# jgsimard/big-dreamer

Hardware: AMD Instinct MI355X
Metric: latent transitions/sec (RSSM + imagination) at batch=50 chunk=50 H=15 (higher is better)
Workload: dtype f32

## Files before the change

### big_dreamer_amd/_cabi.py

```python
from __future__ import annotations

import ctypes as C
import os

import torch

_HERE = os.path.dirname(os.path.abspath(__file__))
LIB_PATH = os.environ.get("BD_LIB") or os.path.join(_HERE, "libbigdreamer_hip.so")

if not os.path.exists(LIB_PATH):
    raise ImportError(
        f"{LIB_PATH} is missing: the MI355X HIP extension has not been built "
        "(run `python -c 'import __graft_entry__ as g; g.build()'`). There is no CPU fallback.")

lib = C.CDLL(LIB_PATH)

BD_MAX_LAYERS = 6
ACT_NONE, ACT_ELU, ACT_ELU_GRAD = 0, 1, 2
ACT_RELU, ACT_RELU_GRAD, ACT_TANH, ACT_TANH_GRAD = 3, 4, 5, 6
CNN_ACTS = {"ELU": (ACT_ELU, ACT_ELU_GRAD), "ReLU": (ACT_RELU, ACT_RELU_GRAD), "Tanh": (ACT_TANH, ACT_TANH_GRAD)}
GRAD_ACTS = (ACT_ELU_GRAD, ACT_RELU_GRAD, ACT_TANH_GRAD)
P = C.c_void_p
F32 = C.c_float
I32 = C.c_int
# ... 197 lines not shown
    "bd_rng_fill": (I32, [C.POINTER(RngFillArgs), P]),
    "bd_philox4x32_10": (I32, [C.POINTER(C.c_uint), C.POINTER(C.c_uint), C.POINTER(C.c_uint)]),
    "bd_actor_entropy_rng": (I32, [C.c_ulonglong, C.c_ulonglong, C.c_uint, P, P, I32, I32, I32, I32, P]),
    "bd_gemm_nt": (I32, [P, I32, P, I32, P, I32, I32, I32, I32, I32, P]),
    "bd_categorical_head_forward": (I32, [P, P, I32, I32, I32, P, P, P]),
    "bd_categorical_head_backward": (I32, [P, P, I32, I32, I32, P, P]),
    "bd_kl_categorical_forward": (I32, [P, P, I32, I32, I32, F32, I32, P, I32, P, P]),
    "bd_kl_categorical_backward": (I32, [P, P, I32, I32, I32, F32, F32, F32, F32, P, I32, P, P, P]),
    "bd_plan_rollout": (I32, [C.POINTER(PlanArgs), P]),
    "bd_cem_refit": (I32, [P, I32, P, I32, I32, I32, I32, I32, P, P, P]),
    "bd_plan_rollout_cat": (I32, [C.POINTER(PlanCatArgs), P]),
    "bd_lambda_return_backward": (I32, [P, F32, I32, I32, F32, F32, P, P, P]),
    "bd_img_heads_supported": (I32, [I32, I32]),
    "bd_img_heads_fwd_bwd": (I32, [C.POINTER(ImgHeadsArgs), P]),
    "bd_actor_reinforce": (I32, [P, P, P, P, P, P, P, I32, I32, I32, F32, F32, F32, I32, P, P, I32, P, P]),
    "bd_actor_reinforce_cat": (I32, [P, P, P, P, P, P, I32, I32, I32, F32, F32, F32, I32, P, P, I32, P, P]),
    "bd_normal_nll": (I32, [P, I32, P, I32, I32, I32, F32, P, I32, P, I32, P, P]),
    "bd_bernoulli_nll": (I32, [P, P, C.c_size_t, F32, P, P, I32, P, P]),
    "bd_kl_forward": (I32, [P, P, P, P, I32, I32, F32, I32, P, I32, P, P]),
    "bd_kl_backward": (I32, [P, P, P, P, I32, I32, F32, F32, F32, F32, P, I32, P, P, P, P, P]),
    "bd_sum": (I32, [P, C.c_size_t, P, I32, P, P]),
    "bd_sumsq": (I32, [P, C.c_size_t, P, I32, P, P]),
    "bd_adam_step": (I32, [P, P, P, P, C.c_size_t, F32, F32, F32, F32, F32, I32, F32, P, I32, P]),
    "bd_polyak": (I32, [P, P, C.c_size_t, F32, P]),
    "bd_replay_gather": (I32, [P, P, I32, I32, P, P]),
    "bd_replay_gather_pixels": (I32, [P, P, I32, I32, I32, P, P, P]),
    "bd_replay_gather_pixels_rng": (I32, [P, P, I32, I32, I32, C.c_ulonglong, C.c_ulonglong, P, P]),
    "bd_reduce_ws_floats": (C.c_size_t, []),
    "bd_conv_gemm": (I32, [C.POINTER(ConvArgs), P]),
    "bd_conv_thin_forward": (I32, [P, I32, I32, I32, I32, I32, P, I32, P, I32, P, P, P]),
    "bd_conv_pack_class": (I32, [P, P, I32, I32, I32, I32, I32, I32, I32, P]),
    "bd_conv_pack_fused": (I32, [P, P, I32, I32, I32, P]),
    "bd_act_backward": (I32, [P, P, C.c_size_t, I32, P]),
    "bd_elu_backward": (I32, [P, P, C.c_size_t, P]),
    "bd_image_layout": (I32, [P, P, I32, I32, I32, I32, P]),
    "bd_colsum_ws_floats": (C.c_size_t, [I32]),
    "bd_colsum": (I32, [P, C.c_size_t, I32, P, P, P]),
}

for _name, (_res, _args) in _SIGS.items():
    _fn = getattr(lib, _name)
    _fn.restype = _res
    _fn.argtypes = _args

EXPORTED = tuple(_SIGS)

# ... 24 lines not shown
```

### big_dreamer_amd/csrc/cabi.hip

```cpp
#include "bd_device.h"
#include "bd_host.h"
#include "bd_rng.h"

namespace bd {
char* err_buf() {
    static thread_local char buf[512] = "";
    return buf;
}

__global__ __launch_bounds__(256) void pack_kernel(const bd_pack_desc* __restrict__ descs) {
    const bd_pack_desc d = descs[blockIdx.y];
    const int No = d.transpose ? d.K : d.N;
    const int Ki = d.transpose ? d.N : d.K;
    const int Nb = (No + 15) >> 4, Kb = (Ki + 15) >> 4;
    const int total = Nb * Kb * 64;
    floatx4* __restrict__ dst = reinterpret_cast<floatx4*>(d.dst);
    for (int e = blockIdx.x * blockDim.x + threadIdx.x; e < total; e += gridDim.x * blockDim.x) {
        const int lane = e & 63, blk = e >> 6;
        const int nb = blk / Kb, kb = blk - nb * Kb;
        const int n = nb * 16 + (lane & 15);
        const int k0 = kb * 16 + 4 * (lane >> 4);
        floatx4 v;
#pragma unroll
        for (int i = 0; i < 4; ++i) {
            const int k = k0 + i;
            float x = 0.f;
            if (n < No && k < Ki) x = d.transpose ? d.src[(size_t)k * d.ld + n] : d.src[(size_t)n * d.ld + k];
            v[i] = x;
        }
        dst[e] = v;
    }
}

__global__ __launch_bounds__(256) void gather_rows_kernel(const float* __restrict__ src, const int64_t* __restrict__ idx,
                                                          int n_idx, int width, float* __restrict__ dst) {
    const size_t total = (size_t)n_idx * width;
    for (size_t e = (size_t)blockIdx.x * blockDim.x + threadIdx.x; e < total; e += (size_t)gridDim.x * blockDim.x) {
        const size_t r = e / width, c = e - r * width;
        dst[e] = src[(size_t)idx[r] * width + c];
    }
}
template <bool RNG>
__global__ __launch_bounds__(256) void gather_pixels_kernel(const unsigned char* __restrict__ src,
                                                            const int64_t* __restrict__ idx, int n_idx, int pixels,
                                                            float inv_q, float inv_b, const float* __restrict__ noise,
                                                            float* __restrict__ dst, Rng rng) {
    const int quads = pixels >> 2;
    const size_t total = (size_t)n_idx * quads;
    for (size_t e = (size_t)blockIdx.x * blockDim.x + threadIdx.x; e < total; e += (size_t)gridDim.x * blockDim.x) {
        const size_t r = e / quads, q = e - r * quads;
        const uchar4 u = reinterpret_cast<const uchar4*>(src + (size_t)idx[r] * pixels)[q];
        floatx4 nz;
        if constexpr (RNG) {
            const Philox4 p = philox4x32_10((uint32_t)e, (uint32_t)(e >> 32), rng.stream, rng.step, rng.k0, rng.k1);
// ... 65 lines not shown
```

### big_dreamer_amd/csrc/reduce.hip

```cpp
#include "bd_device.h"
#include "bd_host.h"
#include "bd_discrete.h"

namespace bd {

constexpr int kRedBlocks = 1024;
constexpr float kHalfLog2Pi = 0.91893853320467274178f;

static inline int red_blocks(size_t n) {
    size_t b = (n + 255) / 256;
    return (int)(b < 1 ? 1 : (b > kRedBlocks ? kRedBlocks : b));
}

__global__ __launch_bounds__(256) void final_sum_kernel(const double* __restrict__ partials, int n,
                                                        float* __restrict__ scalars, int slot) {
    __shared__ double red[kWaves];
    double s = 0.0;
    for (int i = threadIdx.x; i < n; i += blockDim.x) s += partials[i];
    s = block_sum_d(s, red);
    if (threadIdx.x == 0) scalars[slot] = (float)s;
}

template <int MODE>
__global__ __launch_bounds__(256) void sum_kernel(const float* __restrict__ x, size_t n, double* __restrict__ partials) {
    __shared__ double red[kWaves];
// ... 131 lines not shown
    const size_t n = (size_t)M * S;
    for (size_t i = (size_t)blockIdx.x * blockDim.x + threadIdx.x; i < n; i += (size_t)gridDim.x * blockDim.x) {
        const size_t r = i / S, c = i - r * S;
        const float ds = dstate ? dstate[i] : 0.f;
        const float gm = ds + (dmean ? dmean[i] : 0.f);
        const float gs = (dstate ? ds * eps[i] : 0.f) + (dstd ? dstd[i] : 0.f);
        dout[r * 2 * S + c] = gm;
        dout[r * 2 * S + S + c] = gs * sigmoidf(out[r * 2 * S + S + c]);
    }
}

__global__ __launch_bounds__(256) void lambda_fwd_kernel(const float* __restrict__ reward, const float* __restrict__ value,
                                                         int Hm, int N, float disc, float lam, float* __restrict__ ret) {
    const float one_minus = 1.f - lam, dl = disc * lam;
    for (int n = blockIdx.x * blockDim.x + threadIdx.x; n < N; n += gridDim.x * blockDim.x) {
        const float boot = value[(size_t)(Hm - 1) * N + n];
        float last = boot;
        for (int t = Hm - 1; t >= 0; --t) {
            const float next = (t == Hm - 1) ? boot : value[(size_t)(t + 1) * N + n];
            const float inp = reward[(size_t)t * N + n] + disc * next * one_minus;
            last = inp + dl * last;
            ret[(size_t)t * N + n] = last;
        }
    }
}

__global__ __launch_bounds__(256) void lambda_bwd_kernel(const float* __restrict__ dret, float dconst, int Hm, int N,
                                                         float disc, float lam, float* __restrict__ dreward,
                                                         float* __restrict__ dvalue) {
    const float c = disc * lam, w = disc * (1.f - lam);
    for (int n = blockIdx.x * blockDim.x + threadIdx.x; n < N; n += gridDim.x * blockDim.x) {
        float G = 0.f;
        for (int t = 0; t < Hm; ++t) {
            G = (dret ? dret[(size_t)t * N + n] : dconst) + c * G;
            dreward[(size_t)t * N + n] = G;
            if (t == 0 && Hm > 1) dvalue[n] = 0.f;
            if (t < Hm - 1) {
                dvalue[(size_t)(t + 1) * N + n] = G * w;
            } else {
                const float prev = (Hm > 1) ? dvalue[(size_t)t * N + n] : 0.f;
                dvalue[(size_t)t * N + n] = prev + G * w + c * G;
            }
        }
    }
}

// ... 53 lines not shown
        const float w = weight ? weight[i] : 1.f;
        const float adv = ret[i] - (i < N ? base0[i] : value[i - N]);
        const float c = scale * w * adv;
        const size_t j = (size_t)i * A + lane;
        const float norm = valid ? stats[j] : -INFINITY;
        const unsigned long long hot = __ballot(valid && action[j] > 0.5f);
        const int k = hot ? __builtin_ctzll(hot) : 0;
        const float p = disc_probs(norm, valid);
        const float l = __shfl(norm, k, 64);
        float g = c * ((lane == k ? 1.f : 0.f) - p);
        if (write) {
            const float H = disc_entropy(norm, p, valid);
            g += (dentropy * w) * (-p * (norm + H));
        } else if (valid) {
            g += dout[j];
        }
        if (valid) dout[j] = g;
        if (lane == 0) s += (double)(w * l * adv);
    }
    s = block_sum_d(s, red);
    if (threadIdx.x == 0) partials[blockIdx.x] = s;
}

__global__ __launch_bounds__(256) void adam_kernel(float* __restrict__ p, float* __restrict__ g, float* __restrict__ m,
                                                   float* __restrict__ v, size_t n, float beta1, float beta2, float eps,
                                                   float wd, float step_size, float inv_sqrt_bc2, float max_norm,
                                                   const float* __restrict__ scalars, int sqnorm_slot) {
    const float total_norm = sqrtf(scalars[sqnorm_slot]);
    const float q = max_norm / (total_norm + 1e-6f);
    const float coef = q > 1.f ? 1.f : q;
    for (size_t i = (size_t)blockIdx.x * blockDim.x + threadIdx.x; i < n; i += (size_t)gridDim.x * blockDim.x) {
        const float gc = g[i] * coef;
        g[i] = gc;
        const float pi = p[i];
        const float gw = gc + wd * pi;
        const float mi = m[i] + (1.f - beta1) * (gw - m[i]);
        const float vi = v[i] * beta2 + (1.f - beta2) * gw * gw;
        m[i] = mi;
        v[i] = vi;
        const float denom = sqrtf(vi) * inv_sqrt_bc2 + eps;
        p[i] = pi - step_size * (mi / denom);
    }
}

__global__ __launch_bounds__(256) void polyak_kernel(float* __restrict__ t, const float* __restrict__ s, size_t n, float w) {
    for (size_t i = (size_t)blockIdx.x * blockDim.x + threadIdx.x; i < n; i += (size_t)gridDim.x * blockDim.x)
        t[i] = s[i] * w + t[i] * (1.f - w);
}

constexpr int kCatPer = 4;

__device__ __forceinline__ float half_max(float v) {
#pragma unroll
    for (int o = 16; o > 0; o >>= 1) v = fmaxf(v, __shfl_xor(v, o, 64));
    return v;
}
__device__ __forceinline__ float half_sum(float v) {
#pragma unroll
    for (int o = 16; o > 0; o >>= 1) v += __shfl_xor(v, o, 64);
    return v;
}

__device__ __forceinline__ void group_log_softmax(const float* __restrict__ x, int C, int l, float (&lp)[kCatPer]) {
    float m = -INFINITY;
// ... 296 lines not shown
    BD_CHECK_LAUNCH("bd_lambda_return_forward");
    return 0;
}

int bd_lambda_return_backward(const float* dreturns, float dret_const, int Hm, int N, float discount, float lambda_,
                              float* dreward, float* dvalue, void* stream) {
    BD_REQUIRE(dreward && dvalue && Hm > 0 && N > 0, "bd_lambda_return_backward: bad arguments");
    hipLaunchKernelGGL(lambda_bwd_kernel, dim3(red_blocks(N)), dim3(256), 0, (hipStream_t)stream, dreturns, dret_const, Hm,
                       N, discount, lambda_, dreward, dvalue);
    BD_CHECK_LAUNCH("bd_lambda_return_backward");
    return 0;
}

int bd_adam_step(float* p, float* g, float* m, float* v, size_t n, float lr, float beta1, float beta2, float eps,
                 float weight_decay, int step, float max_norm, const float* scalars, int sqnorm_slot, void* stream) {
    BD_REQUIRE(p && g && m && v && scalars && n > 0 && step >= 1, "bd_adam_step: bad arguments");
    const double bc1 = 1.0 - pow((double)beta1, step), bc2 = 1.0 - pow((double)beta2, step);
    hipLaunchKernelGGL(adam_kernel, dim3(red_blocks(n)), dim3(256), 0, (hipStream_t)stream, p, g, m, v, n, beta1, beta2,
                       eps, weight_decay, (float)(lr / bc1), (float)(1.0 / sqrt(bc2)), max_norm, scalars, sqnorm_slot);
    BD_CHECK_LAUNCH("bd_adam_step");
    return 0;
}

int bd_polyak(float* target, const float* src, size_t n, float weight, void* stream) {
    BD_REQUIRE(target && src && n > 0, "bd_polyak: bad arguments");
    hipLaunchKernelGGL(polyak_kernel, dim3(red_blocks(n)), dim3(256), 0, (hipStream_t)stream, target, src, n, weight);
    BD_CHECK_LAUNCH("bd_polyak");
    return 0;
}

static inline int cat_blocks(size_t units) {
    size_t b = (units + 7) / 8;
    return (int)(b < 1 ? 1 : (b > (size_t)kRedBlocks ? (size_t)kRedBlocks : b));
}

int bd_categorical_head_forward(const float* logits, const float* q_noise, int rows, int D, int C, float* state,
                                float* probs, void* stream) {
    BD_REQUIRE(logits && q_noise && state && probs && rows > 0 && D > 0, "bd_categorical_head_forward: bad arguments");
    BD_REQUIRE(C > 0 && C <= 32 * kCatPer, "bd_categorical_head_forward: %d classes (max %d)", C, 32 * kCatPer);
    const size_t groups = (size_t)rows * D;
    hipLaunchKernelGGL(cat_head_fwd_kernel, dim3(cat_blocks(groups)), dim3(256), 0, (hipStream_t)stream, logits, q_noise,
                       groups, C, state, probs);
    BD_CHECK_LAUNCH("bd_categorical_head_forward");
    return 0;
}

// ... 38 lines not shown
```

### big_dreamer_amd/engine.py

```python
from __future__ import annotations

import collections.abc
import ctypes as C
import math
import os
import weakref
from typing import Dict, List, Optional, Tuple

import numpy as np
import torch

from . import _cabi as cabi
from .parallel import DataParallel
from .params import ParamGroup, _adam_state_dict, _load_adam_state_dict
from .synth import CNN_ACTIVATIONS, DENSE_LAYERS, MODEL_MODULES, Dims, model_modules, param_shapes

lib = cabi.lib
ptr = cabi.ptr

DEFAULT_HP = dict(
    kl_balance=0.8, kl_loss_weight=0.1, free_nats=3.0, grad_clip_norm=100.0, discount=0.995, disclam=0.95,
    model_learning_rate=2e-4, actor_learning_rate=4e-5, value_learning_rate=1e-4, adam_epsilon=1e-5,
    weight_decay=1e-6, entropy_weight=1e-5, polyak_avg=1.0, min_std_dev=0.1, discount_weight=5.0,
    gradient_mixing=-1,
)

ACT_RAW_INIT_STD = float(torch.log(torch.exp(torch.tensor(5.0)) - 1))
ACT_MIN_STD = 1e-4
ACT_MEAN_SCALE = 5.0

SLOT_OBS, SLOT_REW, SLOT_KL, SLOT_RET, SLOT_ENT, SLOT_VAL, SLOT_GN_MODEL, SLOT_GN_ACTOR, SLOT_GN_CRITIC = range(9)
SLOT_DISC, SLOT_WOBJ = 9, 10
SLOT_RF = 11
N_SLOTS = 16


def check_gradient_mixing(value) -> float:
    try:
        rho = float(value)
    except (TypeError, ValueError):
        raise ValueError(f"gradient_mixing must be -1 or a number in [0, 1], got {value!r}") from None
    if not (rho == -1 or 0.0 <= rho <= 1.0):
        raise ValueError(f"gradient_mixing must be -1 or a number in [0, 1], got {value!r}")
    return rho


def check_cnn_activation(value) -> str:
    if value not in CNN_ACTIVATIONS:
        raise ValueError(f"cnn_activation_function must be one of {CNN_ACTIVATIONS}, got {value!r}")
    return value


def check_dense_activation(value) -> str:
    if value != "ELU":
        raise NotImplementedError("the HIP path implements the reference default activation (ELU)")
    return value
# ... 135 lines not shown
            tiny = torch.zeros(4, dtype=torch.float32, device=self.dev)
            for g in (None, "model", "actor", "critic"):
                self.dp.allreduce_sum_(tiny, g)
            torch.cuda.synchronize(self.dev)
        d = dims
        shapes = param_shapes(d)
        self.groups = {
            "model": ParamGroup([(m, n, s) for m in model_modules(d) for n, s in shapes[m]], self.dev,
                                conv_storage=self.pixel),
            "actor": ParamGroup([("actor", n, s) for n, s in shapes["actor"]], self.dev),
            "critic": ParamGroup([("critic", n, s) for n, s in shapes["critic"]], self.dev),
            "critic_target": ParamGroup([("critic_target", n, s) for n, s in shapes["critic"]], self.dev, False),
        }
        self._mod_group = {m: "model" for m in model_modules(d)}
        self._mod_group.update(actor="actor", critic="critic", critic_target="critic_target")
        if params is not None:
            self.load_params(params)
        self.scalars = torch.zeros(N_SLOTS, dtype=torch.float32, device=self.dev)
        self.red_ws = torch.zeros(int(lib.bd_reduce_ws_floats()), dtype=torch.float32, device=self.dev)
        self._wgrad_ws = torch.zeros(1, dtype=torch.float32, device=self.dev)
        self._wgrad_ws_side = torch.zeros(1, dtype=torch.float32, device=self.dev)
        self._wgrad_ws_early = torch.zeros(1, dtype=torch.float32, device=self.dev)
        self.red_ws_side = torch.zeros(int(lib.bd_reduce_ws_floats()), dtype=torch.float32, device=self.dev)
        self._wbatch = {"model": WgradBatch(self, "model"), "model_early": WgradBatch(self, "model_early", "_wgrad_ws_early"),
                        "actor": WgradBatch(self, "actor", "_wgrad_ws_bh"),
                        "critic": WgradBatch(self, "critic", "_wgrad_ws_side")}
        self._side = _engine_stream(self.dev, "side", int(os.environ.get("BD_SIDE_PRIO", "0")))
        self.heads_fused = (os.environ.get("BD_HEADS_FUSED", "1") != "0" and not self.d.categorical
                            and bool(lib.bd_img_heads_supported(self.d.Be + self.d.S, self.d.Hd)))
        self._s_early = _engine_stream(self.dev, "early", int(os.environ.get("BD_EARLY_PRIO", "0")))
        self.pipeline = os.environ.get("BD_PIPELINE", "1") != "0"
        self._s_wm = _engine_stream(self.dev, "wm", int(os.environ.get("BD_WM_PRIO", "-1")))
        bh_prio = int(os.environ.get("BD_BH_PRIO", "0" if self.pixel else "-1"))
        self._s_bh = _engine_stream(self.dev, "bh", bh_prio)
        self._ev_bh_wm_free: Optional[torch.cuda.Event] = None
        self._ev_bh_done: List[Optional[torch.cuda.Event]] = [None, None]
        self._ev_cr_done: List[Optional[torch.cuda.Event]] = [None, None]
        shared_comm = not all(g in self.dp.groups for g in ("model", "actor", "critic"))
        self.defer_opt = (world_size > 1 and shared_comm) or os.environ.get("BD_DEFER_OPT", "0") == "1"
        if os.environ.get("BD_FORCE_DP", "0") == "1" and torch.distributed.is_initialized():
            self.dp.force = True
            self.defer_opt = shared_comm or os.environ.get("BD_DEFER_OPT", "0") == "1"
        if (world_size > 1 or self.dp.force) and torch.cuda.current_stream(self.dev) == torch.cuda.default_stream(self.dev):
            self._main_stream = _engine_stream(self.dev, "main", 0)
            torch.cuda.set_stream(self._main_stream)
        self._pending_opt: List[tuple] = []
# ... 168 lines not shown
        if d.discrete_actions:
            add("actor", "a4", Wa4, tr=True)
        else:
            add("actor", "a4m", Wa4[:A], tr=True)
            add("actor", "a4s", Wa4[A:], tr=True)
            add("actor", "a4", Wa4, fwd=False, tr=True)

        self.pk: Dict[str, torch.Tensor] = {}
        self._pack_tables = {}
        for group, lst in ent.items():
            total = sum(cabi.packed_floats(*(v.shape if not tr else v.shape[::-1])) for _, v, tr in lst)
            store = torch.zeros(total, dtype=torch.float32, device=self.dev)
            descs = (cabi.PackDesc * len(lst))()
            off = 0
            for i, (key, v, tr) in enumerate(lst):
                N, K = v.shape
                n = cabi.packed_floats(N, K)
                self.pk[key] = store[off:off + n]
                descs[i] = cabi.PackDesc(v.data_ptr(), self.pk[key].data_ptr(), v.stride(0), N, K, int(tr))
                off += n
            raw = torch.frombuffer(bytearray(bytes(descs)), dtype=torch.uint8).to(self.dev)
            self._pack_tables[group] = (raw, len(lst), store)

    def pack(self, group: str) -> None:
        raw, n, _ = self._pack_tables[group]
        cabi.check(lib.bd_pack_weights(raw.data_ptr(), n, cabi.stream()))
        for dst, src, grp in self._plain.values():
            if grp == group:
                dst.copy_(src.t())
        if group == "model" and self.conv is not None:
            self.conv.pack()

    def _dense_spec(self, mod: str, prefix: str, in_width: int, out_width: int):
        sizes = [in_width] + [self.d.Hd] * DENSE_LAYERS + [out_width]
        return [(f"{prefix}{l}", self.W(mod, f"model.{2 * l}.bias"), sizes[l + 1], sizes[l],
                 cabi.ACT_ELU if l < DENSE_LAYERS else cabi.ACT_NONE) for l in range(DENSE_LAYERS + 1)]

    def mlp_forward(self, M, in0, ld0, w0, layers, saves, out, ldo, in1=None, ld1=0, w1=0, raw_packs=False,
                    gather=None) -> None:
        a = cabi.MlpFwdArgs()
        a.M, a.in0, a.ld0, a.w0 = M, ptr(in0), ld0, w0
        a.in1, a.ld1, a.w1 = ptr(in1), ld1, w1
        if gather is not None:
            a.gidx, a.gWT, a.gD, a.gC = ptr(gather[0]), ptr(gather[1]), gather[2], gather[3]
        a.n_layers = len(layers)
        for i, (key, bias, N, K, act) in enumerate(layers):
            a.layer[i] = cabi.Layer(ptr(key if raw_packs else self.pk[key]), ptr(bias), N, K, act,
                                    ptr(saves[i]) if saves else None)
        a.out, a.ldo = ptr(out), ldo
# ... 21 lines not shown
        cabi.check(lib.bd_wgrad(ptr(dpre), ldp, ptr(act), lda, M, N, K, ptr(dW), ldw, ptr(db), int(accumulate),
                                ptr(self._wgrad_ws), self._wgrad_ws.numel(), cabi.stream()))

    def _dense_wgrads(self, batch: "WgradBatch", mod: str, M: int, dpres, inp, ld_in, saves, sizes) -> None:
        for l in range(len(sizes) - 1):
            act, lda = (inp, ld_in) if l == 0 else (saves[l - 1], sizes[l])
            batch.add(dpres[l], sizes[l + 1], act, lda, M, sizes[l + 1], sizes[l],
                      self.G(mod, f"model.{2 * l}.weight"), sizes[l], self.G(mod, f"model.{2 * l}.bias"))

    def _allreduce(self, t: torch.Tensor, key: Optional[str] = None) -> None:
        self.dp.allreduce_sum_(t, key)

    def optimizer_step(self, group: str, slot: int, lr: float, red_ws: Optional[torch.Tensor] = None,
                       rec: Optional[_LogRecord] = None) -> None:
        g = self.groups[group]
        red_ws = self.red_ws if red_ws is None else red_ws
        self._allreduce(g.grad, group)
        g.step += 1
        hp = self.hp
        ov = self._opt_over.get(group)
        if ov:
            lr = ov.get("lr", lr)
        eps, wd = (ov or {}).get("eps", hp["adam_epsilon"]), (ov or {}).get("weight_decay", hp["weight_decay"])
        cabi.check(lib.bd_sumsq(ptr(g.grad), g.numel, ptr(self.scalars), slot, ptr(red_ws), cabi.stream()))
        cabi.check(lib.bd_adam_step(ptr(g.flat), ptr(g.grad), ptr(g.m), ptr(g.v), g.numel, lr, 0.9, 0.999,
                                    eps, wd, g.step, hp["grad_clip_norm"],
                                    ptr(self.scalars), slot, cabi.stream()))
        self.pack(group)
        rec = rec if rec is not None else self._cur_rec
        if rec is not None:
            self._snapshot(rec, _LogRecord.ROW[group])

    def _new_record(self) -> _LogRecord:
        if len(self._log_ring) < 8:
            self._log_ring.append(_LogRecord())
            rec = self._log_ring[-1]
        else:
            rec = self._log_ring[self._log_i]
            self._log_i = (self._log_i + 1) % 8
            owner = rec.owner() if rec.owner is not None else None
            if owner is not None and owner._vals is None:
                owner.resolve()
        rec.events = [None, None, None]
        rec.owner, rec.counts = None, None
        return rec

    def _snapshot(self, rec: _LogRecord, row: int) -> None:
        rec.host[row, :N_SLOTS].copy_(self.scalars, non_blocking=True)
        if row == 0 and self._obs_ws is not None and self._obs_err_off is not None:
            rec.host[row, N_SLOTS:].copy_(self._cluster_error_word(), non_blocking=True)
        ev = torch.cuda.Event()
        ev.record(torch.cuda.current_stream())
        rec.events[row] = ev

    def _resolve_record(self, rec: _LogRecord) -> Dict[str, float]:
        if any(p[6] is rec for p in self._pending_opt):
            if self.world_size > 1:
                raise RuntimeError("log dict of a train step whose actor / critic updates are still queued (data-parallel "
                                   "deferred schedule): call train_step(), update_critic(), update_belief_and_act() or "
                                   "flush_optimizers() on EVERY rank before reading it -- reading a log dict never issues "
                                   "collectives")
            self.flush_optimizers()
        for row in rec.need:
            assert rec.events[row] is not None, "log record read before its step was queued"
            rec.events[row].synchronize()
        h = rec.host.numpy()
        s = h[0, :N_SLOTS].copy()
        for slot in (SLOT_RET, SLOT_ENT, SLOT_GN_ACTOR, SLOT_WOBJ, SLOT_RF):
            s[slot] = h[1, slot]
        for slot in (SLOT_VAL, SLOT_GN_CRITIC):
            s[slot] = h[2, slot]
        self._raise_on_cluster_error(int(h[0, N_SLOTS:].view(np.uint32)[0]))
        return self._logs_from(s, rec.counts)

    def _cluster_error_word(self) -> torch.Tensor:
        w = self._obs_ws[self._obs_err_off:self._obs_err_off + 1]
        if self.world_size <= 1:
            return w
        flag = (w.view(torch.int32) != 0).to(torch.float32)
        self._allreduce(flag, "model")
        return torch.where(flag > 0, torch.full_like(flag, 3).to(torch.int32), torch.zeros_like(flag).to(torch.int32)).view(torch.float32)

    def _raise_on_cluster_error(self, word: int) -> None:
        if word:
            off = self._obs_err_off
            self._obs_ws[off:off + 1].zero_()
            which = "+".join(n for b, n in ((1, "forward"), (2, "backward")) if word & b)
            raise RuntimeError(f"bigdreamer_hip: a member of the cluster observe scan timed out waiting for its peers "
                               f"({which} scan): the step's posteriors / gradients are wrong (BD_OBS_CLUSTER=0 selects "
                               "the single-workgroup scan)")

    def update_critic(self) -> None:
        self.flush_optimizers()
        self.join()
        t, s = self.groups["critic_target"], self.groups["critic"]
# ... 672 lines not shown
            wts.view(Hm, N).copy_(torch.cumprod(arr, 0))
            if mix is None:
                dret = self.buf("dret_w", Mi)
                torch.mul(wts, -inv_mi, out=dret)
            elif dyn:
                dret = self.buf("dret_w", Mi)
                torch.mul(wts, -mix * inv_mi, out=dret)
        fused = dyn and self.heads_fused
        if dyn:
            d_r, d_v = self.buf("d_ir_out", Mi), self.buf("d_iv_out", Mi)
            dconst = -inv_mi if mix is None else -mix * inv_mi
            difeat = self.buf("difeat", Mi, F)
        if fused:
            cabi.check(lib.bd_lambda_return_backward(ptr(dret), dconst, Hm, N, hp["discount"], hp["disclam"], ptr(d_r),
                                                     ptr(d_v), st))
            r_out, v_out = self.buf("ir_out", Mi, 1), self.buf("iv_out", Mi, 1)
            with self.span("img_heads_bwd"):
                self.img_heads_fused(Mi, ifeat, d_r, d_v, r_out, v_out, difeat)
        else:
            with self.span("img_heads_fwd"):
                r_out, r_acts, r_layers = self.dense_forward("reward_model", "rew", "ir", ifeat, F, Mi, 1, sidx=isidx)
                v_out, v_acts, v_layers = self.dense_forward("critic_target", "tgt", "iv", ifeat, F, Mi, 1, sidx=isidx)
        returns = self.buf(ptag + "returns", Mi)
        cabi.check(lib.bd_lambda_return_forward(ptr(r_out), ptr(v_out), Hm, N, hp["discount"], hp["disclam"], ptr(returns), st))
        cabi.check(lib.bd_sum(ptr(returns), Mi, sc, SLOT_RET, ws, st))
        cabi.check(lib.bd_sum(ptr(ent), Mi, sc, SLOT_ENT, ws, st))
        if d.use_discount:
            ew_ = hp["entropy_weight"] if hp["entropy_weight"] != -1 else 0.0
            if mix is None:
                self.scalars[SLOT_WOBJ] = (wts * (returns + ew_ * ent)).sum()
            else:
                self.scalars[SLOT_WOBJ] = (wts * (mix * returns + ew_ * ent)).sum()
        if par is not None:
            ev_ret = torch.cuda.Event()
            ev_ret.record(torch.cuda.current_stream())
            with torch.cuda.stream(self._side):
                self._side.wait_event(ev_ret)
                self._critic_phase(ifeat, returns, Mi, F, inv_mi, self.red_ws_side, isidx, wts)
                self._ev_cr_done[par] = torch.cuda.Event()
                self._ev_cr_done[par].record(self._side)
        dentropy = -hp["entropy_weight"] * inv_mi if hp["entropy_weight"] != -1 else 0.0
        d_apre, d_aout = self.buf("d_actor_pre", DENSE_LAYERS, Mi, d.Hd), self.buf("d_actor_out", Mi, d.actor_out)
        sv_actor = self._buf["sv_actor"]
        actor_chain = os.environ.get("BD_ACTOR_BWD_CHAIN", "1") == "1" or mix is not None or d.discrete_actions
        if dyn:
            if not fused:
                cabi.check(lib.bd_lambda_return_backward(ptr(dret), dconst, Hm, N, hp["discount"], hp["disclam"],
                                                         ptr(d_r), ptr(d_v), st))
                with self.span("img_heads_bwd"):
# ... 138 lines not shown
```

### include/bigdreamer_hip.h

```cpp
#ifndef BIGDREAMER_HIP_H
#define BIGDREAMER_HIP_H

#include <stddef.h>
#include <stdint.h>

#ifdef __cplusplus
extern "C" {
#endif

#define BD_MAX_LAYERS 6
#define BD_ACT_NONE 0
#define BD_ACT_ELU 1
#define BD_ACT_ELU_GRAD 2
#define BD_ACT_RELU 3
#define BD_ACT_RELU_GRAD 4
#define BD_ACT_TANH 5
#define BD_ACT_TANH_GRAD 6

const char* bd_last_error(void);
int bd_version(void);

typedef struct {
    const float* src;
    float* dst;
// ... 190 lines not shown
    int N, Hm, Be, S, A, Hd;
    const float* wt_embed_s; const float* wt_embed_a;
    const float* wt_ir; const float* wt_iz; const float* wt_in;
    const float* wt_hr; const float* wt_hz; const float* wt_hn;
    const float* wt_p1; const float* wt_p2m; const float* wt_p2s;
    const float* wt_a[3];
    const float* wt_a4m; const float* wt_a4s;
    const float* start_feat; const float* feat; const float* prior_std; const float* action;
    const float* eps_action; const float* eps_prior;
    const float* sv_actor; const float* sv_act_stats; const float* sv_x; const float* sv_gates;
    const float* sv_p;
    float min_std;
    const float* dfeat;
    float dentropy;
    float* d_actor_pre;
    float* d_actor_out;
    const float* ent_weight;
    int discrete_actions;
} bd_imagine_bwd_args;
int bd_imagine_backward(const bd_imagine_bwd_args* a, void* stream);

int bd_lambda_return_forward(const float* reward, const float* value, int Hm, int N, float discount,
                             float lambda_, float* returns, void* stream);
int bd_lambda_return_backward(const float* dreturns, float dret_const, int Hm, int N, float discount,
                              float lambda_, float* dreward, float* dvalue, void* stream);

#define BD_HEAD_HIDDEN 4
typedef struct {
    const float* w[BD_HEAD_HIDDEN];
    const float* wt[BD_HEAD_HIDDEN];
    const float* b[BD_HEAD_HIDDEN];
    const float* w_out;
    const float* b_out;
    const float* dout;
    float* out;
} bd_img_head;
typedef struct {
    int M, F, Hd;
    const float* x;
    bd_img_head head[2];
    float* dx;
} bd_img_heads_args;
int bd_img_heads_supported(int F, int Hd);
int bd_img_heads_fwd_bwd(const bd_img_heads_args* a, void* stream);

int bd_actor_reinforce(const float* eps_action, const float* act_us, const float* act_stats, const float* returns,
// ... 175 lines not shown
    float* actions;
    float* returns;
    float* feat;
    unsigned char* sidx;
} bd_plan_cat_args;
int bd_plan_rollout_cat(const bd_plan_cat_args* a, void* stream);

int bd_normal_nll(const float* pred, int ldp, const float* target, int ldt, int rows, int D,
                  float grad_scale, float* dpred, int ldd, float* scalars, int slot, float* ws, void* stream);
int bd_bernoulli_nll(const float* logits, const float* target, size_t n, float grad_scale, float* dlogits, float* scalars,
                     int slot, float* ws, void* stream);

int bd_kl_forward(const float* qm, const float* qs, const float* pm, const float* ps, int rows, int S,
                  float free_nats, int sum_form, float* scalars, int slot, float* ws, void* stream);
int bd_kl_backward(const float* qm, const float* qs, const float* pm, const float* ps, int rows, int S,
                   float free_nats, float kl_balance, float weight, float inv_count, const float* scalars,
                   int slot, float* dqm, float* dqs, float* dpm, float* dps, void* stream);
int bd_sum(const float* x, size_t n, float* scalars, int slot, float* ws, void* stream);
int bd_sumsq(const float* x, size_t n, float* scalars, int slot, float* ws, void* stream);

int bd_adam_step(float* p, float* g, float* m, float* v, size_t n, float lr, float beta1, float beta2,
                 float eps, float weight_decay, int step, float max_norm, const float* scalars,
                 int sqnorm_slot, void* stream);
int bd_polyak(float* target, const float* src, size_t n, float weight, void* stream);

int bd_replay_gather(const float* src, const int64_t* idx, int n_idx, int width, float* dst, void* stream);

int bd_replay_gather_pixels(const unsigned char* src, const int64_t* idx, int n_idx, int pixels, int bit_depth,
                            const float* noise, float* dst, void* stream);
int bd_replay_gather_pixels_rng(const unsigned char* src, const int64_t* idx, int n_idx, int pixels, int bit_depth,
                                unsigned long long seed, unsigned long long step, float* dst, void* stream);

size_t bd_reduce_ws_floats(void);

#ifdef __cplusplus
}
#endif
#endif
```

Before: 13.33 million.

## Fuse optimiser sumsq, Adam and weight packing into one grid-barrier kernel

```diff
diff --git a/big_dreamer_amd/_cabi.py b/big_dreamer_amd/_cabi.py
--- a/big_dreamer_amd/_cabi.py
+++ b/big_dreamer_amd/_cabi.py
@@ -243,6 +243,11 @@
     "bd_sum": (I32, [P, C.c_size_t, P, I32, P, P]),
     "bd_sumsq": (I32, [P, C.c_size_t, P, I32, P, P]),
     "bd_adam_step": (I32, [P, P, P, P, C.c_size_t, F32, F32, F32, F32, F32, I32, F32, P, I32, P]),
+    "bd_update_ws_floats": (C.c_size_t, []),
+    "bd_update_blocks": (I32, []),
+    "bd_update_fused": (I32, [P, P, P, P, C.c_size_t, F32, F32, F32, F32, F32, I32, F32, P, I32, P, I32, I32, P, P]),
+    "bd_lambda_sums_ws_floats": (C.c_size_t, []),
+    "bd_lambda_return_forward_sums": (I32, [P, P, P, I32, I32, F32, F32, P, P, I32, I32, P, P]),
     "bd_polyak": (I32, [P, P, C.c_size_t, F32, P]),
     "bd_replay_gather": (I32, [P, P, I32, I32, P, P]),
     "bd_replay_gather_pixels": (I32, [P, P, I32, I32, I32, P, P, P]),
diff --git a/big_dreamer_amd/csrc/bd_pack.h b/big_dreamer_amd/csrc/bd_pack.h
--- /dev/null
+++ b/big_dreamer_amd/csrc/bd_pack.h
@@ -0,0 +1,30 @@
+#pragma once
+#include "bd_device.h"
+
+namespace bd {
+
+__device__ __forceinline__ void pack_slice(const bd_pack_desc& d, int bx, int nbx) {
+    const int No = d.transpose ? d.K : d.N;
+    const int Ki = d.transpose ? d.N : d.K;
+    const int Nb = (No + 15) >> 4, Kb = (Ki + 15) >> 4;
+    const int total = Nb * Kb * 64;
+    const float* src = d.src;
+    floatx4* dst = reinterpret_cast<floatx4*>(d.dst);
+    for (int e = bx * blockDim.x + threadIdx.x; e < total; e += nbx * blockDim.x) {
+        const int lane = e & 63, blk = e >> 6;
+        const int nb = blk / Kb, kb = blk - nb * Kb;
+        const int n = nb * 16 + (lane & 15);
+        const int k0 = kb * 16 + 4 * (lane >> 4);
+        floatx4 v;
+#pragma unroll
+        for (int i = 0; i < 4; ++i) {
+            const int k = k0 + i;
+            float x = 0.f;
+            if (n < No && k < Ki) x = d.transpose ? src[(size_t)k * d.ld + n] : src[(size_t)n * d.ld + k];
+            v[i] = x;
+        }
+        dst[e] = v;
+    }
+}
+
+}
diff --git a/big_dreamer_amd/csrc/cabi.hip b/big_dreamer_amd/csrc/cabi.hip
--- a/big_dreamer_amd/csrc/cabi.hip
+++ b/big_dreamer_amd/csrc/cabi.hip
@@ -1,5 +1,6 @@
 #include "bd_device.h"
 #include "bd_host.h"
+#include "bd_pack.h"
 #include "bd_rng.h"
 
 namespace bd {
@@ -10,26 +11,7 @@
 
 __global__ __launch_bounds__(256) void pack_kernel(const bd_pack_desc* __restrict__ descs) {
     const bd_pack_desc d = descs[blockIdx.y];
-    const int No = d.transpose ? d.K : d.N;
-    const int Ki = d.transpose ? d.N : d.K;
-    const int Nb = (No + 15) >> 4, Kb = (Ki + 15) >> 4;
-    const int total = Nb * Kb * 64;
-    floatx4* __restrict__ dst = reinterpret_cast<floatx4*>(d.dst);
-    for (int e = blockIdx.x * blockDim.x + threadIdx.x; e < total; e += gridDim.x * blockDim.x) {
-        const int lane = e & 63, blk = e >> 6;
-        const int nb = blk / Kb, kb = blk - nb * Kb;
-        const int n = nb * 16 + (lane & 15);
-        const int k0 = kb * 16 + 4 * (lane >> 4);
-        floatx4 v;
-#pragma unroll
-        for (int i = 0; i < 4; ++i) {
-            const int k = k0 + i;
-            float x = 0.f;
-            if (n < No && k < Ki) x = d.transpose ? d.src[(size_t)k * d.ld + n] : d.src[(size_t)n * d.ld + k];
-            v[i] = x;
-        }
-        dst[e] = v;
-    }
+    pack_slice(d, blockIdx.x, gridDim.x);
 }
 
 __global__ __launch_bounds__(256) void gather_rows_kernel(const float* __restrict__ src, const int64_t* __restrict__ idx,
diff --git a/big_dreamer_amd/csrc/reduce.hip b/big_dreamer_amd/csrc/reduce.hip
--- a/big_dreamer_amd/csrc/reduce.hip
+++ b/big_dreamer_amd/csrc/reduce.hip
@@ -1,6 +1,8 @@
 #include "bd_device.h"
 #include "bd_host.h"
 #include "bd_discrete.h"
+#include "bd_cluster.h"
+#include "bd_pack.h"
 
 namespace bd {
 
@@ -178,6 +180,62 @@
             last = inp + dl * last;
             ret[(size_t)t * N + n] = last;
         }
+    }
+}
+
+template <class Store>
+__device__ __forceinline__ float lambda_scan(const float* __restrict__ reward, const float* __restrict__ value, int Hm, int N,
+                                             int n, int t0, float disc, float one_minus, float dl, Store&& store) {
+#pragma clang fp contract(off)
+    const float boot = value[(size_t)(Hm - 1) * N + n];
+    float last = (reward[(size_t)(Hm - 1) * N + n] + (disc * boot) * one_minus) + dl * boot;
+    store(Hm - 1, last);
+    for (int t = Hm - 2; t >= t0; --t) {
+        const float inp = __builtin_fmaf(one_minus, disc * value[(size_t)(t + 1) * N + n], reward[(size_t)t * N + n]);
+        last = __builtin_fmaf(dl, last, inp);
+        store(t, last);
+    }
+    return last;
+}
+
+__global__ __launch_bounds__(256) void lambda_fwd_sums_kernel(const float* __restrict__ reward,
+                                                              const float* __restrict__ value,
+                                                              const float* __restrict__ ent, int Hm, int N, float disc,
+                                                              float lam, float* ret, double* partials, unsigned* ticket,
+                                                              float* scalars, int slot_ret, int slot_ent) {
+    __shared__ double red[kWaves];
+    __shared__ int is_last;
+    const float one_minus = 1.f - lam, dl = disc * lam;
+    for (int n = blockIdx.x * blockDim.x + threadIdx.x; n < N; n += gridDim.x * blockDim.x) {
+        lambda_scan(reward, value, Hm, N, n, 0, disc, one_minus, dl, [&](int t, float r) { ret[(size_t)t * N + n] = r; });
+    }
+    const size_t Mi = (size_t)Hm * N;
+    double sr = 0.0, se = 0.0;
+    for (size_t i = (size_t)blockIdx.x * blockDim.x + threadIdx.x; i < Mi; i += (size_t)gridDim.x * blockDim.x) {
+        const int t0 = (int)(i / N), n = (int)(i - (size_t)t0 * N);
+        sr += (double)lambda_scan(reward, value, Hm, N, n, t0, disc, one_minus, dl, [](int, float) {});
+        se += (double)ent[i];
+    }
+    sr = block_sum_d(sr, red);
+    se = block_sum_d(se, red);
+    if (threadIdx.x == 0) {
+        partials[blockIdx.x] = sr;
+        partials[kRedBlocks + blockIdx.x] = se;
+        __builtin_amdgcn_fence(__ATOMIC_RELEASE, "agent");
+        asm volatile("s_waitcnt vmcnt(0)" ::: "memory");
+        const unsigned old = __hip_atomic_fetch_add(ticket, 1u, __ATOMIC_RELAXED, __HIP_MEMORY_SCOPE_AGENT);
+        is_last = (old == gridDim.x - 1);
+        if (old == gridDim.x - 1) __hip_atomic_store(ticket, 0u, __ATOMIC_RELAXED, __HIP_MEMORY_SCOPE_AGENT);
+    }
+    __syncthreads();
+    if (!is_last) return;
+    __builtin_amdgcn_fence(__ATOMIC_ACQUIRE, "agent");
+    const int nb = gridDim.x;
+    for (int which = 0; which < 2; ++which) {
+        double s = 0.0;
+        for (int i = threadIdx.x; i < nb; i += blockDim.x) s += partials[which * kRedBlocks + i];
+        s = block_sum_d(s, red);
+        if (threadIdx.x == 0) scalars[which ? slot_ent : slot_ret] = (float)s;
     }
 }
 
@@ -277,6 +335,20 @@
     if (threadIdx.x == 0) partials[blockIdx.x] = s;
 }
 
+__device__ __forceinline__ void adam_elem(float* p, float* g, float* m, float* v, size_t i, float coef, float beta1,
+                                          float beta2, float eps, float wd, float step_size, float inv_sqrt_bc2) {
+#pragma clang fp contract(off)
+    const float gi = g[i], pi = p[i], m0 = m[i];
+    g[i] = gi * coef;
+    const float gw = __builtin_fmaf(gi, coef, wd * pi);
+    const float mi = __builtin_fmaf(1.f - beta1, gw - m0, m0);
+    const float vi = v[i] * beta2 + ((1.f - beta2) * gw) * gw;
+    m[i] = mi;
+    v[i] = vi;
+    const float denom = __builtin_fmaf(sqrtf(vi), inv_sqrt_bc2, eps);
+    p[i] = __builtin_fmaf(-step_size, mi / denom, pi);
+}
+
 __global__ __launch_bounds__(256) void adam_kernel(float* __restrict__ p, float* __restrict__ g, float* __restrict__ m,
                                                    float* __restrict__ v, size_t n, float beta1, float beta2, float eps,
                                                    float wd, float step_size, float inv_sqrt_bc2, float max_norm,
@@ -285,16 +357,76 @@
     const float q = max_norm / (total_norm + 1e-6f);
     const float coef = q > 1.f ? 1.f : q;
     for (size_t i = (size_t)blockIdx.x * blockDim.x + threadIdx.x; i < n; i += (size_t)gridDim.x * blockDim.x) {
-        const float gc = g[i] * coef;
-        g[i] = gc;
-        const float pi = p[i];
-        const float gw = gc + wd * pi;
-        const float mi = m[i] + (1.f - beta1) * (gw - m[i]);
-        const float vi = v[i] * beta2 + (1.f - beta2) * gw * gw;
-        m[i] = mi;
-        v[i] = vi;
-        const float denom = sqrtf(vi) * inv_sqrt_bc2 + eps;
-        p[i] = pi - step_size * (mi / denom);
+        adam_elem(p, g, m, v, i, coef, beta1, beta2, eps, wd, step_size, inv_sqrt_bc2);
+    }
+}
+
+constexpr int kUpdBlocks = 128;
+static_assert((kUpdBlocks & (kUpdBlocks - 1)) == 0, "the ticket arithmetic needs a power of two");
+constexpr int kUpdHeaderFloats = 16;
+
+__device__ __forceinline__ void update_grid_barrier(unsigned* ticket, unsigned* err) {
+    asm volatile("s_waitcnt vmcnt(0)" ::: "memory");
+    __syncthreads();
+    if (threadIdx.x == 0) {
+        __builtin_amdgcn_fence(__ATOMIC_RELEASE, "agent");
+        asm volatile("s_waitcnt vmcnt(0)" ::: "memory");
+        const unsigned old = __hip_atomic_fetch_add(ticket, 1u, __ATOMIC_RELAXED, __HIP_MEMORY_SCOPE_AGENT);
+        const unsigned target = (old & ~(unsigned)(kUpdBlocks - 1)) + kUpdBlocks;
+        unsigned spins = 0;
+        while ((int)(__hip_atomic_load(ticket, __ATOMIC_RELAXED, __HIP_MEMORY_SCOPE_AGENT) - target) < 0) {
+            if (++spins > kSpinLimit) {
+                __hip_atomic_fetch_or(err, 1u, __ATOMIC_RELAXED, __HIP_MEMORY_SCOPE_AGENT);
+                break;
+            }
+            __builtin_amdgcn_s_sleep(2);
+        }
+    }
+    __syncthreads();
+    __builtin_amdgcn_fence(__ATOMIC_ACQUIRE, "agent");
+}
+
+__global__ __launch_bounds__(256) void update_fused_kernel(float* p, float* g, float* m, float* v, size_t n, int nb,
+                                                           float beta1, float beta2, float eps, float wd, float step_size,
+                                                           float inv_sqrt_bc2, float max_norm,
+                                                           const bd_pack_desc* __restrict__ descs, int n_descs,
+                                                           float* scalars, int slot, int err_slot, float* ws) {
+    __shared__ double red[kWaves];
+    __shared__ float sq_sh;
+    unsigned* ticket = reinterpret_cast<unsigned*>(ws);
+    unsigned* err = reinterpret_cast<unsigned*>(scalars + err_slot);
+    double* partials = reinterpret_cast<double*>(ws + kUpdHeaderFloats);
+    for (int vb = blockIdx.x; vb < nb; vb += gridDim.x) {
+        double s = 0.0;
+        for (size_t i = (size_t)vb * blockDim.x + threadIdx.x; i < n; i += (size_t)nb * blockDim.x) {
+            const float x = g[i];
+            s += (double)x * x;
+        }
+        s = block_sum_d(s, red);
+        if (threadIdx.x == 0) partials[vb] = s;
+    }
+    update_grid_barrier(ticket, err);
+    {
+        double s = 0.0;
+        for (int i = threadIdx.x; i < nb; i += blockDim.x) s += partials[i];
+        s = block_sum_d(s, red);
+        if (threadIdx.x == 0) {
+            sq_sh = (float)s;
+            if (blockIdx.x == 0) scalars[slot] = (float)s;
+        }
+        __syncthreads();
+    }
+    const float total_norm = sqrtf(sq_sh);
+    const float q = max_norm / (total_norm + 1e-6f);
+    const float coef = q > 1.f ? 1.f : q;
+    for (size_t i = (size_t)blockIdx.x * blockDim.x + threadIdx.x; i < n; i += (size_t)gridDim.x * blockDim.x) {
+        adam_elem(p, g, m, v, i, coef, beta1, beta2, eps, wd, step_size, inv_sqrt_bc2);
+    }
+    if (n_descs <= 0) return;
+    update_grid_barrier(ticket, err);
+    for (int it = blockIdx.x; it < 16 * n_descs; it += gridDim.x) {
+        const bd_pack_desc d = descs[it >> 4];
+        pack_slice(d, it & 15, 16);
     }
 }
 
@@ -637,6 +769,38 @@
     return 0;
 }
 
+size_t bd_lambda_sums_ws_floats(void) { return 16 + 4 * (size_t)kRedBlocks; }
+
+int bd_lambda_return_forward_sums(const float* reward, const float* value, const float* ent, int Hm, int N, float discount,
+                                  float lambda_, float* returns, float* scalars, int slot_ret, int slot_ent, float* ws,
+                                  void* stream) {
+    BD_REQUIRE(reward && value && ent && returns && scalars && ws && Hm > 0 && N > 0 && slot_ret >= 0 && slot_ent >= 0,
+               "bd_lambda_return_forward_sums: bad arguments");
+    BD_REQUIRE((size_t)Hm * N <= (size_t)INT32_MAX, "bd_lambda_return_forward_sums: %d x %d elements", Hm, N);
+    const int nb = red_blocks((size_t)Hm * N);
+    hipLaunchKernelGGL(lambda_fwd_sums_kernel, dim3(nb), dim3(256), 0, (hipStream_t)stream, reward, value, ent, Hm, N,
+                       discount, lambda_, returns, (double*)(ws + 16), (unsigned*)ws, scalars, slot_ret, slot_ent);
+    BD_CHECK_LAUNCH("bd_lambda_return_forward_sums");
+    return 0;
+}
+
+size_t bd_update_ws_floats(void) { return kUpdHeaderFloats + 2 * (size_t)kRedBlocks; }
+int bd_update_blocks(void) { return kUpdBlocks; }
+
+int bd_update_fused(float* p, float* g, float* m, float* v, size_t n, float lr, float beta1, float beta2, float eps,
+                    float weight_decay, int step, float max_norm, const bd_pack_desc* descs, int n_descs, float* scalars,
+                    int sqnorm_slot, int err_slot, float* ws, void* stream) {
+    BD_REQUIRE(p && g && m && v && scalars && ws && n > 0 && step >= 1 && sqnorm_slot >= 0 && err_slot >= 0 &&
+                   err_slot != sqnorm_slot, "bd_update_fused: bad arguments");
+    BD_REQUIRE(n_descs >= 0 && (n_descs == 0 || descs != nullptr), "bd_update_fused: %d descriptors without a table", n_descs);
+    const double bc1 = 1.0 - pow((double)beta1, step), bc2 = 1.0 - pow((double)beta2, step);
+    hipLaunchKernelGGL(update_fused_kernel, dim3(kUpdBlocks), dim3(256), 0, (hipStream_t)stream, p, g, m, v, n,
+                       red_blocks(n), beta1, beta2, eps, weight_decay, (float)(lr / bc1), (float)(1.0 / sqrt(bc2)), max_norm,
+                       descs, n_descs, scalars, sqnorm_slot, err_slot, ws);
+    BD_CHECK_LAUNCH("bd_update_fused");
+    return 0;
+}
+
 int bd_polyak(float* target, const float* src, size_t n, float weight, void* stream) {
     BD_REQUIRE(target && src && n > 0, "bd_polyak: bad arguments");
     hipLaunchKernelGGL(polyak_kernel, dim3(red_blocks(n)), dim3(256), 0, (hipStream_t)stream, target, src, n, weight);
diff --git a/big_dreamer_amd/engine.py b/big_dreamer_amd/engine.py
--- a/big_dreamer_amd/engine.py
+++ b/big_dreamer_amd/engine.py
@@ -32,6 +32,7 @@
 SLOT_OBS, SLOT_REW, SLOT_KL, SLOT_RET, SLOT_ENT, SLOT_VAL, SLOT_GN_MODEL, SLOT_GN_ACTOR, SLOT_GN_CRITIC = range(9)
 SLOT_DISC, SLOT_WOBJ = 9, 10
 SLOT_RF = 11
+SLOT_UPD_ERR = 15
 N_SLOTS = 16
 
 
@@ -213,6 +214,10 @@
         self._wgrad_ws_side = torch.zeros(1, dtype=torch.float32, device=self.dev)
         self._wgrad_ws_early = torch.zeros(1, dtype=torch.float32, device=self.dev)
         self.red_ws_side = torch.zeros(int(lib.bd_reduce_ws_floats()), dtype=torch.float32, device=self.dev)
+        self.update_fused = os.environ.get("BD_UPDATE_FUSED", "1") != "0"
+        self._upd_ws = {k: torch.zeros(int(lib.bd_update_ws_floats()), dtype=torch.float32, device=self.dev)
+                        for k in ("model", "actor", "critic")}
+        self._lam_ws = torch.zeros(int(lib.bd_lambda_sums_ws_floats()), dtype=torch.float32, device=self.dev)
         self._wbatch = {"model": WgradBatch(self, "model"), "model_early": WgradBatch(self, "model_early", "_wgrad_ws_early"),
                         "actor": WgradBatch(self, "actor", "_wgrad_ws_bh"),
                         "critic": WgradBatch(self, "critic", "_wgrad_ws_side")}
@@ -427,9 +432,10 @@
             raw = torch.frombuffer(bytearray(bytes(descs)), dtype=torch.uint8).to(self.dev)
             self._pack_tables[group] = (raw, len(lst), store)
 
-    def pack(self, group: str) -> None:
-        raw, n, _ = self._pack_tables[group]
-        cabi.check(lib.bd_pack_weights(raw.data_ptr(), n, cabi.stream()))
+    def pack(self, group: str, images: bool = True) -> None:
+        if images:
+            raw, n, _ = self._pack_tables[group]
+            cabi.check(lib.bd_pack_weights(raw.data_ptr(), n, cabi.stream()))
         for dst, src, grp in self._plain.values():
             if grp == group:
                 dst.copy_(src.t())
@@ -497,11 +503,18 @@
         if ov:
             lr = ov.get("lr", lr)
         eps, wd = (ov or {}).get("eps", hp["adam_epsilon"]), (ov or {}).get("weight_decay", hp["weight_decay"])
-        cabi.check(lib.bd_sumsq(ptr(g.grad), g.numel, ptr(self.scalars), slot, ptr(red_ws), cabi.stream()))
-        cabi.check(lib.bd_adam_step(ptr(g.flat), ptr(g.grad), ptr(g.m), ptr(g.v), g.numel, lr, 0.9, 0.999,
-                                    eps, wd, g.step, hp["grad_clip_norm"],
-                                    ptr(self.scalars), slot, cabi.stream()))
-        self.pack(group)
+        if self.update_fused:
+            raw, n, _ = self._pack_tables[group]
+            cabi.check(lib.bd_update_fused(ptr(g.flat), ptr(g.grad), ptr(g.m), ptr(g.v), g.numel, lr, 0.9, 0.999, eps, wd,
+                                           g.step, hp["grad_clip_norm"], raw.data_ptr(), n, ptr(self.scalars), slot,
+                                           SLOT_UPD_ERR, ptr(self._upd_ws[group]), cabi.stream()))
+            self.pack(group, images=False)
+        else:
+            cabi.check(lib.bd_sumsq(ptr(g.grad), g.numel, ptr(self.scalars), slot, ptr(red_ws), cabi.stream()))
+            cabi.check(lib.bd_adam_step(ptr(g.flat), ptr(g.grad), ptr(g.m), ptr(g.v), g.numel, lr, 0.9, 0.999,
+                                        eps, wd, g.step, hp["grad_clip_norm"],
+                                        ptr(self.scalars), slot, cabi.stream()))
+            self.pack(group)
         rec = rec if rec is not None else self._cur_rec
         if rec is not None:
             self._snapshot(rec, _LogRecord.ROW[group])
@@ -546,6 +559,10 @@
         for slot in (SLOT_VAL, SLOT_GN_CRITIC):
             s[slot] = h[2, slot]
         self._raise_on_cluster_error(int(h[0, N_SLOTS:].view(np.uint32)[0]))
+        if any(int(h[row, SLOT_UPD_ERR:SLOT_UPD_ERR + 1].view(np.uint32)[0]) for row in rec.need):
+            self.scalars[SLOT_UPD_ERR:SLOT_UPD_ERR + 1].zero_()
+            raise RuntimeError("bigdreamer_hip: a workgroup of a fused optimiser update timed out at its grid barrier: "
+                               "the parameters are wrong (BD_UPDATE_FUSED=0 selects the separate launches)")
         return self._logs_from(s, rec.counts)
 
     def _cluster_error_word(self) -> torch.Tensor:
@@ -1264,9 +1281,13 @@
                 r_out, r_acts, r_layers = self.dense_forward("reward_model", "rew", "ir", ifeat, F, Mi, 1, sidx=isidx)
                 v_out, v_acts, v_layers = self.dense_forward("critic_target", "tgt", "iv", ifeat, F, Mi, 1, sidx=isidx)
         returns = self.buf(ptag + "returns", Mi)
-        cabi.check(lib.bd_lambda_return_forward(ptr(r_out), ptr(v_out), Hm, N, hp["discount"], hp["disclam"], ptr(returns), st))
-        cabi.check(lib.bd_sum(ptr(returns), Mi, sc, SLOT_RET, ws, st))
-        cabi.check(lib.bd_sum(ptr(ent), Mi, sc, SLOT_ENT, ws, st))
+        if self.update_fused and not d.use_discount and mix is None:
+            cabi.check(lib.bd_lambda_return_forward_sums(ptr(r_out), ptr(v_out), ptr(ent), Hm, N, hp["discount"], hp["disclam"],
+                                                         ptr(returns), sc, SLOT_RET, SLOT_ENT, ptr(self._lam_ws), st))
+        else:
+            cabi.check(lib.bd_lambda_return_forward(ptr(r_out), ptr(v_out), Hm, N, hp["discount"], hp["disclam"], ptr(returns), st))
+            cabi.check(lib.bd_sum(ptr(returns), Mi, sc, SLOT_RET, ws, st))
+            cabi.check(lib.bd_sum(ptr(ent), Mi, sc, SLOT_ENT, ws, st))
         if d.use_discount:
             ew_ = hp["entropy_weight"] if hp["entropy_weight"] != -1 else 0.0
             if mix is None:
diff --git a/include/bigdreamer_hip.h b/include/bigdreamer_hip.h
--- a/include/bigdreamer_hip.h
+++ b/include/bigdreamer_hip.h
@@ -236,6 +236,10 @@
 
 int bd_lambda_return_forward(const float* reward, const float* value, int Hm, int N, float discount,
                              float lambda_, float* returns, void* stream);
+size_t bd_lambda_sums_ws_floats(void);
+int bd_lambda_return_forward_sums(const float* reward, const float* value, const float* ent, int Hm, int N,
+                                  float discount, float lambda_, float* returns, float* scalars, int slot_ret,
+                                  int slot_ent, float* ws, void* stream);
 int bd_lambda_return_backward(const float* dreturns, float dret_const, int Hm, int N, float discount,
                               float lambda_, float* dreward, float* dvalue, void* stream);
 
@@ -457,6 +461,11 @@
 int bd_adam_step(float* p, float* g, float* m, float* v, size_t n, float lr, float beta1, float beta2,
                  float eps, float weight_decay, int step, float max_norm, const float* scalars,
                  int sqnorm_slot, void* stream);
+size_t bd_update_ws_floats(void);
+int bd_update_blocks(void);
+int bd_update_fused(float* p, float* g, float* m, float* v, size_t n, float lr, float beta1, float beta2, float eps,
+                    float weight_decay, int step, float max_norm, const bd_pack_desc* descs, int n_descs,
+                    float* scalars, int sqnorm_slot, int err_slot, float* ws, void* stream);
 int bd_polyak(float* target, const float* src, size_t n, float weight, void* stream);
 
 int bd_replay_gather(const float* src, const int64_t* idx, int n_idx, int width, float* dst, void* stream);
```

Result: slower. 12.92 million (-3.1%).
